# tirtho109/parallel_AMG

Measured on AMD Instinct MI355X. Metric: V-cycle iters/sec + fine-SpMV HBM GB/s, 3D Poisson 128M dofs at 1/2/4/8 GPU, higher is better.
Workload: dtype f64; 1 GPU; poisson3d 512^3 fp64, SA-AMG V(1,1) weighted-Jacobi, 1 part(s); n=134217728, nnz_fine=937951232, levels=6, max_coarse=1000, parallelism=row-slab partition p1

## Files before the change

### parallel_amg_amd/csrc/kernels.hip

```cpp

#include "pamg_device.h"
#include "div_rn.h"

namespace pamg {
namespace {

__device__ __forceinline__ int wave_incl_scan(int v) {
    const int lane = threadIdx.x & 63, rl = lane & 15;
    int t;
    t = __builtin_amdgcn_mov_dpp(v, 0x111, 0xf, 0xf, false);
    if (rl >= 1) v += t;
    t = __builtin_amdgcn_mov_dpp(v, 0x112, 0xf, 0xf, false);
    if (rl >= 2) v += t;
    t = __builtin_amdgcn_mov_dpp(v, 0x114, 0xf, 0xf, false);
    if (rl >= 4) v += t;
    t = __builtin_amdgcn_mov_dpp(v, 0x118, 0xf, 0xf, false);
    if (rl >= 8) v += t;
    t = __builtin_amdgcn_mov_dpp(v, 0x142, 0xf, 0xf, false);
    if (lane & 16) v += t;
    t = __builtin_amdgcn_mov_dpp(v, 0x143, 0xf, 0xf, false);
    if (lane >= 32) v += t;
    return v;
}

// ... 1964 lines not shown
#pragma unroll
            for (int q = 0; q < NS; ++q) {
                const int L = (int)(pw[q] & 7u);
#pragma unroll
                for (int k = 0; k < LM; ++k) {
                    const uint32_t c = (pw[q] >> (3 + 3 * k)) & 7u;
                    const int c01 = c & 1u ? an[q][0] : r[q].a0;
                    const int c23 = c & 1u ? an[q][2] : an[q][1];
                    const int c45 = c & 1u ? r[q].am : an[q][3];
                    const int c03 = c & 2u ? c23 : c01;
                    const int c47 = c & 2u ? r[q].ap : c45;
                    col[q][k] = c & 4u ? c47 : c03;
                    xv[q][k] = x[k < L ? col[q][k] : col[q][0]];
                }
            }
        };
        const int lm = 3 + (__any(lmax > 3) ? 1 : 0) + (__any(lmax > 4) ? 1 : 0) + (__any(lmax > 5) ? 1 : 0) +
                       (__any(lmax > 6) ? 1 : 0);
        switch (lm) {
            case 3: loads(std::integral_constant<int, 3>{}); break;
            case 4: loads(std::integral_constant<int, 4>{}); break;
            case 5: loads(std::integral_constant<int, 5>{}); break;
            case 6: loads(std::integral_constant<int, 6>{}); break;
            default: loads(std::integral_constant<int, 7>{}); break;
        }
#pragma unroll
        for (int q = 0; q < NS; ++q) {
            const int in = min(zs[q] + j + 1, zl[q]) * M + ixy, z2 = min(za[q] + 2, nz - 1);
            if constexpr (CP) nrec[q] = make_uint2((uint32_t)cid[in], 0u);
            else nrec[q] = rec[in];
            np0[q] = 0.0;
            np1[q] = 0.0;
            if constexpr (OP == OP_RESID || OP == OP_JACOBI) np0[q] = b[in];
            if constexpr (OP == OP_PROLONG) np0[q] = y[in];
            if constexpr (OP == OP_JACOBI) np1[q] = x[in];
            ap2[q] = anc[z2 * M + ixy];
            rg2[q] = 0;
            if (rxy >= 0) rg2[q] = anc[z2 * M + rxy];
        }
#pragma unroll
        for (int q = 0; q < NS; ++q) {
            const int i = min(zs[q] + j, zl[q]) * M + ixy, L = (int)(pw[q] & 7u);
            uint64_t rr;
            if constexpr (CP) rr = r[q].rec.x < (uint32_t)npat ? lw[r[q].rec.x] : 0ull;
            else rr = (((uint64_t)r[q].rec.y << 32) | r[q].rec.x) >> 10;
            double s = 0.0, dg = 0.0;
#pragma unroll
            for (int k = 0; k < kPncMaxLen; ++k) {
                const bool ok = k < L;
                const double v = lv[(uint32_t)(rr >> (7 * k)) & 127u];
                const double p = v * xv[q][k];
                const double t = s + p;
                s = ok ? t : s;
                if constexpr (OP == OP_JACOBI) dg = ok && col[q][k] == i ? v : dg;
            }
            double out;
            if constexpr (OP == OP_SPMV) {
                out = s;
            } else if constexpr (OP == OP_RESID) {
                out = r[q].p0 - s;
            } else if constexpr (OP == OP_JACOBI) {
                const double uu = r[q].p0 - s;
                const double v = omega * uu;
                const double w = v / dg;
                out = r[q].p1 + w;
            } else {
                out = r[q].p0 + s;
            }
            const bool in = CP ? r[q].rec.x != (uint32_t)kPncCombSkip : (r[q].rec.x & 1023u) != (uint32_t)kPncSkip;
            if (zs[q] + j < ze[q] && in) y[i] = out;
            r[q].rec = nrec[q];
            r[q].p0 = np0[q];
            r[q].p1 = np1[q];
            r[q].am = r[q].a0;
            r[q].a0 = r[q].ap;
            r[q].ap = ap2[q];
            r[q].rg = rg2[q];
            za[q] = min(za[q] + 1, nz - 1);
        }
        __syncthreads();
    }
}

template <int OP>
__global__ __launch_bounds__(kBlock) void k_rows_long(
    const int* __restrict__ rows, const int* __restrict__ rowptr, const int* __restrict__ col,
    const double* __restrict__ val, const double* __restrict__ x, const double* __restrict__ b,
    double* __restrict__ y, double omega, double c1 = 0.0, const double* __restrict__ xold = nullptr) {
    __shared__ double lprod[kBlock + 8];
    __shared__ double ldiag;
    const int tid = threadIdx.x;
    const int r = rows[blockIdx.x];
    const int z0 = rowptr[r], z1 = rowptr[r + 1];
    double s = 0.0;
    for (int base = z0; base < z1; base += kBlock) {
        const int k = base + tid;
        double p = 0.0;
        if (k < z1) {
            const int c = col[k];
            const double v = val[k];
            p = v * x[c];
            if constexpr (kDiagOp<OP>) {
                if (c == r) ldiag = v;
            }
        }
        lprod[tid] = p;
        __syncthreads();
        if (tid == 0) s = row_sum_lds(lprod, 0, min(kBlock, z1 - base), s);
        __syncthreads();
    }
    if constexpr (OP == OP_CHEB) {
        if (tid == 0) epilogue<OP>(r, s, x, b, y, omega, ldiag, c1, xold);
    } else {
        if (tid == 0) epilogue<OP>(r, s, x, b, y, omega, OP == OP_JACOBI ? ldiag : 0.0);
    }
}

__global__ __launch_bounds__(kBlock) void k_cheb_update(int64_t n, const uint8_t* __restrict__ mask, int mask_bytes,
                                                        const uint8_t* __restrict__ ids,
                                                        const uint32_t* __restrict__ mtab, uint32_t in_flag,
                                                        const double* __restrict__ diag, const double* __restrict__ x,
                                                        const double* __restrict__ xold, double* __restrict__ y,
                                                        double c1, double c2) {
    for (int64_t i = blockIdx.x * (int64_t)kBlock + threadIdx.x; i < n; i += (int64_t)gridDim.x * kBlock) {
        const uint32_t m = ids ? mtab[ids[i]]
                               : (mask_bytes == 1 ? (uint32_t)mask[i] : (uint32_t)reinterpret_cast<const uint16_t*>(mask)[i]);
        if (!(m & in_flag)) continue;
        y[i] = cheb_step(y[i], x[i], xold ? xold[i] : 0.0, diag[i], c1, c2);
    }
}

__global__ void k_jacobi_zero(int64_t n, const double* __restrict__ b,
                              const double* __restrict__ diag, double omega,
                              double* __restrict__ y) {
    for (int64_t i = blockIdx.x * (int64_t)blockDim.x + threadIdx.x; i < n;
         i += (int64_t)gridDim.x * blockDim.x) {
        const double u = b[i] - 0.0;
        const double v = omega * u;
        const double w = v / diag[i];
        y[i] = 0.0 + w;
    }
}

constexpr int kGemvChunk = 1024;
__global__ __launch_bounds__(kBlock) void k_dense_gemv(int64_t n_rows, int64_t n,
                                                       int64_t row0,
                                                       const double* __restrict__ ainv,
                                                       const double* __restrict__ b,
                                                       double* __restrict__ y) {
    __shared__ __attribute__((aligned(16))) double lp_all[kBlock / 64][kGemvChunk + 8];
    const int w = threadIdx.x >> 6, lane = threadIdx.x & 63;
    const int64_t i = (int64_t)blockIdx.x * (kBlock / 64) + w;
    if (i >= n_rows) return;
    const double* a = ainv + (row0 + i) * n;
    double* lp = lp_all[w];
    double s = 0.0;
    for (int64_t c = 0; c < n; c += kGemvChunk) {
        const int m = (int)((n - c) < kGemvChunk ? (n - c) : kGemvChunk);
#pragma unroll
        for (int q = 0; q < kGemvChunk / 64; ++q) {
            const int j = lane + 64 * q;
            if (j < m) {
                const double p = a[c + j] * b[c + j];
                lp[j] = p;
            }
        }
// ... 338 lines not shown
template <int OP>
bool launch_sym_zm(const pamg_mat& A, const double* x, const double* b, double* y, double omega, hipStream_t s,
                   Cheb ch = Cheb{}) {
    const SymDia& sd = A.sym;
    if (!(sd.nu == 3 && sd.vd_n && sd.tb_ok && !sd.tb_part && options().sym_zm && sd.plane0 == 0 &&
          (int64_t)sd.nbands * sd.band >= A.nrows && A.nrows == (int64_t)sd.tb.nx * sd.tb.ny * sd.tb.nz &&
          A.nrows % 2 == 0))
        return false;
    TbGeom g = sd.tb;
    const int tiles = g.tiles_x * g.tiles_y;
    int zc = options().zm_chunks > 0 ? options().zm_chunks : std::min((1024 + tiles - 1) / tiles, g.nz / 16);
    zc = std::max(1, std::min(zc, g.nz));
    g.zlen = (g.nz + zc - 1) / zc;
    g.zchunks = (g.nz + g.zlen - 1) / g.zlen;
    const int gr = (tiles * g.zchunks + 7) / 8 * 8;
    k_sym_zm<OP><<<gr, kZmThreads, 0, s>>>((int)A.nrows, sd.d_tid, sd.d_vtab, sd.d_mtab, sd.vd_n, g, x, b, y, omega,
                                           ch.c1, ch.xold);
    return true;
}

template <int OP, int NU>
void launch_sym_nu(const pamg_mat& A, const double* x, const double* b, double* y, double omega, hipStream_t s) {
    const SymDia& sd = A.sym;
    const int grid = sd.nbands * 8 * sd.eighth;
    if constexpr (NU == 3) {
        if (launch_sym_zm<OP>(A, x, b, y, omega, s)) return;
    }
    if (sd.vd_n) {
        const int ch = NU <= 3 ? options().symd_chunks : 1;
        const int g = 8 * ((sd.nbands * sd.eighth + ch - 1) / ch);
        if constexpr (NU <= 3) {
            if (ch == 2) {
                k_rows_symd<OP, NU, 2><<<g, kBlock, 0, s>>>((int)A.nrows, (int)A.nrows, sd.d_tid, sd.d_vtab,
                                                            sd.d_mtab, sd.vd_n, sd, x, b, y, omega);
                return;
            }
            if (ch == 4) {
                k_rows_symd<OP, NU, 4><<<g, kBlock, 0, s>>>((int)A.nrows, (int)A.nrows, sd.d_tid, sd.d_vtab,
                                                            sd.d_mtab, sd.vd_n, sd, x, b, y, omega);
                return;
            }
        }
        k_rows_symd<OP, NU><<<grid, kBlock, 0, s>>>((int)A.nrows, (int)A.nrows, sd.d_tid, sd.d_vtab, sd.d_mtab,
                                                  sd.vd_n, sd, x, b, y, omega);
        return;
    }
    if (sd.rpl == 2) {
        k_rows_sym2<OP, NU><<<grid, kBlock, 0, s>>>((int)A.nrows, (int)A.nrows, sd.d_mask, sd.d_diag, sd.d_upper,
                                                  sd.ld, sd, x, b, y, omega);
        return;
    }
    k_rows_sym<OP, NU><<<grid, kBlock, 0, s>>>((int)A.nrows, (int)A.nrows, sd.d_mask, sd.d_diag, sd.d_upper, sd.ld,
                                             sd, x, b, y, omega);
}

template <int OP>
void launch_sym(const pamg_mat& A, const double* x, const double* b, double* y, double omega, hipStream_t s,
                Cheb ch = Cheb{}) {
    if constexpr (OP == OP_PROLONG) {
        return;
    } else if constexpr (OP == OP_CHEB) {
        if (launch_sym_zm<OP_CHEB>(A, x, b, y, omega, s, ch)) return;
        launch_sym<OP_RESID>(A, x, b, y, 0.0, s);
        launch_cheb_update(A, x, ch.xold, y, ch.c1, omega, s);
    } else {
        switch (A.sym.nu) {
            case 1: launch_sym_nu<OP, 1>(A, x, b, y, omega, s); break;
            case 2: launch_sym_nu<OP, 2>(A, x, b, y, omega, s); break;
            case 3: launch_sym_nu<OP, 3>(A, x, b, y, omega, s); break;
            case 4: launch_sym_nu<OP, 4>(A, x, b, y, omega, s); break;
            case 5: launch_sym_nu<OP, 5>(A, x, b, y, omega, s); break;
            case 6: launch_sym_nu<OP, 6>(A, x, b, y, omega, s); break;
            default: launch_sym_nu<OP, 7>(A, x, b, y, omega, s); break;
        }
    }
}

constexpr int kPncZlen = 32, kPncStreams = 2;

template <int OP>
void launch_pnc(const pamg_mat& A, const double* x, const double* b, double* y, double omega, hipStream_t s) {
    const PncSet& P = A.pnc;
    const int zlen = std::min(kPncZlen, P.nz);
    const int nxb = P.nx * P.ny / 256, units = nxb * ((P.nz + zlen - 1) / zlen);
    auto go = [&](auto kern) {
        kern<<<(units + 7) / 8 * 8, 256, 0, s>>>((int)A.nrows, P.nx, P.nx * P.ny, P.nz, zlen, P.d_anc, P.d_rec, P.d_cid,
                                                P.d_pvals, P.d_ptab, P.npat, P.d_vtab, P.nval, x, b, y, omega);
    };
    if (options().pnc == 1 && pnc_tiled(P.nx, P.ny)) {
        if (P.d_cid) go(k_rows_pnct<OP, kPncStreams, true, kPncTx, kPncTy>);
        else go(k_rows_pnct<OP, kPncStreams, false, kPncTx, kPncTy>);
    } else {
        if (P.d_cid) go(k_rows_pnc<OP, kPncStreams, true>);
        else go(k_rows_pnc<OP, kPncStreams, false>);
    }
}

template <int OP>
void launch_rpat(const pamg_mat& A, const double* x, const double* b, double* y, double omega, hipStream_t s) {
    const RpatSet& R = A.rpat;
    const int grid = (int)((R.ngroups + 7) / 8 * 8);
    auto go = [&](auto kern) {
        kern<<<grid, kEllGroup, 0, s>>>((int)A.nrows, R.d_gorder, R.d_anc, R.d_pid, R.d_pmeta, R.npat, R.d_pent, R.nent,
                                        R.d_vtab, R.nval, (int)R.ngroups, x, b, y, omega);
    };
    go(k_rows_rpat<OP, 8>);
}

template <int OP, int FUSE>
void launch_bsr(const pamg_mat& A, const double* x, const double* b, double* y, double omega, hipStream_t s, Cheb ch);

template <int OP>
void launch_rows_op(const pamg_mat& A, const TileSet& ts, const double* x, const double* b,
                    double* y, double omega, hipStream_t s, Cheb ch = Cheb{}) {
    if (ts.bsr) launch_bsr<OP, 0>(A, x, b, y, omega, s, ch);
    if (ts.sym) launch_sym<OP>(A, x, b, y, omega, s, ch);
    if (ts.ell) {
        const EllSet& E = A.ell;
        const int grid = (int)((E.ngroups + 7) / 8 * 8);
        auto go = [&](auto kern) {
            kern<<<grid, kEllGroup, 0, s>>>((int)A.nrows, E.d_gorder, E.d_anc, E.d_smeta, E.d_ci, E.d_vi, E.d_len,
                                            E.d_gmeta, E.d_otab, E.d_vtab, (int)E.ngroups, x, b, y, omega, ch.c1,
                                            ch.xold);
        };
        if (E.win) {
            const int win = std::max(E.max_window, 128);
            const int gather_all = (reinterpret_cast<uintptr_t>(x) & 15) != 0 ? 1 : 0;
            const int npairs = gather_all ? 0 : E.npairs, nrest = (int)E.ngroups - 2 * npairs;
            auto gow = [&](auto kern, int span, int g0, int n, int wn) {
                const size_t bytes = sizeof(double) * (size_t)(wn + 256 * span) + sizeof(uint16_t) * 4 * 256 * span;
                kern<<<(n + 7) / 8 * 8, span * kEllGroup, bytes, s>>>(
                    (int)A.nrows, E.d_gslices, E.d_smeta, E.d_ci, E.d_cid, E.d_len, E.d_dpos, E.d_gmeta, E.d_otab,
                    E.d_vtab, E.d_wmeta, E.d_chunks, E.d_lof, wn, gather_all, E.d_pairs, g0, n, x, b, y, omega, ch.c1,
                    ch.xold);
            };
            if (npairs > 0) {
                const int wu = std::max(E.max_union, 128);
                if (E.cls) gow(k_rows_ellw<OP, true, 2>, 2, 0, npairs, wu);
                else gow(k_rows_ellw<OP, false, 2>, 2, 0, npairs, wu);
            }
            if (nrest > 0) {
                if (E.cls) gow(k_rows_ellw<OP, true>, 1, 2 * npairs, nrest, win);
                else gow(k_rows_ellw<OP, false>, 1, 2 * npairs, nrest, win);
            }
        } else if (E.d_anc) {
            if (E.paired) go(k_rows_ell<OP, true, true>);
            else go(k_rows_ell<OP, true, false>);
        } else {
            if (E.paired) go(k_rows_ell<OP, false, true>);
            else go(k_rows_ell<OP, false, false>);
        }
    }
    if constexpr (OP != OP_CHEB) {
        if (ts.pnc) launch_pnc<OP>(A, x, b, y, omega, s);
        if (ts.rpat) launch_rpat<OP>(A, x, b, y, omega, s);
    }
    if (ts.n_short > 0) {
        if (ts.tile_nnz == 1024) launch_tile<OP, 1024>(A, ts, x, b, y, omega, s, ch);
        else if (ts.tile_nnz == 4096) launch_tile<OP, 4096>(A, ts, x, b, y, omega, s, ch);
        else launch_tile<OP, 2048>(A, ts, x, b, y, omega, s, ch);
    }
    if (ts.n_long > 0)
        k_rows_long<OP><<<ts.n_long, kBlock, 0, s>>>(ts.d_long, A.d_rowptr, A.d_col, A.d_val, x,
                                                     b, y, omega, ch.c1, ch.xold);
}


__global__ __launch_bounds__(kBlock) void k_pcg_alpha(int np, const double* __restrict__ partials, PcgScalars* S) {
    if (S->done) return;
    __shared__ double lds[kBlock / 64];
    double v = 0.0;
    for (int i = threadIdx.x; i < np; i += kBlock) v += partials[i];
    const double s = block_sum(v, lds);
    if (threadIdx.x == 0) {
        S->pq = s;
        S->alpha = S->rz / s;
    }
// ... 339 lines not shown
```

### parallel_amg_amd/csrc/matrix.hip

```cpp
#include <algorithm>
#include <array>
#include <atomic>
#include <chrono>
#include <cstdint>
#include <cstdio>
#include <cstdlib>
#include <cstring>
#include <functional>
#include <iterator>
#include <memory>
#include <mutex>
#include <new>
#include <thread>
#include <utility>
#include <vector>

#include "pamg_device.h"
#include "pamg_host.h"
#include "ell_span.h"

namespace {

int host_threads() {
    static const int n = [] {
// ... 91 lines not shown
    int dev = 0, cus = 0;
    if (hipGetDevice(&dev) != hipSuccess ||
        hipDeviceGetAttribute(&cus, hipDeviceAttributeMultiprocessorCount, dev) != hipSuccess || cus <= 0)
        return 256;
    return cus;
}

std::vector<int> column_reuse_gaps(const PtrVec& rp, const IdxVec& ci, int64_t nrows,
                                   int64_t ncols) {
    std::vector<int> gap(ncols, 0);
    const int nch = (int)std::min<int64_t>(host_threads(), std::max<int64_t>(1, nrows / 65536));
    std::vector<int64_t> r0(nch + 1);
    for (int t = 0; t <= nch; ++t) r0[t] = nrows * t / nch;
    auto each_chunk = [nch](const std::function<void(int)>& f) {
        std::vector<std::thread> th;
        for (int t = 0; t < nch; ++t) th.emplace_back([&f, t] { f(t); });
        for (auto& x : th) x.join();
    };
    std::vector<int> lo(nch, INT32_MAX), hi(nch, -1);
    each_chunk([&](int t) {
        int a = INT32_MAX, b = -1;
        for (int64_t k = rp[r0[t]]; k < rp[r0[t + 1]]; ++k)
            if (ci[k] < ncols) {
                a = std::min(a, ci[k]);
                b = std::max(b, ci[k]);
            }
        lo[t] = a;
        hi[t] = b;
    });
    int64_t span = 0;
    for (int t = 0; t < nch; ++t) span += hi[t] >= lo[t] ? (int64_t)hi[t] - lo[t] + 1 : 0;
    if (nch == 1 || span > 2 * ncols + 65536) {
        std::vector<int> last(ncols, -1);
        for (int64_t i = 0; i < nrows; ++i)
            for (int64_t k = rp[i]; k < rp[i + 1]; ++k) {
                const int c = ci[k];
                if (c < ncols) {
                    if (last[c] >= 0) gap[c] = std::max(gap[c], (int)i - last[c]);
                    last[c] = (int)i;
                }
            }
        return gap;
    }
    std::vector<std::vector<int>> first(nch), last(nch), cgap(nch);
    each_chunk([&](int t) {
        if (hi[t] < lo[t]) return;
        const int64_t w = (int64_t)hi[t] - lo[t] + 1;
        first[t].assign(w, -1);
        last[t].assign(w, -1);
        cgap[t].assign(w, 0);
        int* f = first[t].data();
        int* l = last[t].data();
        int* g = cgap[t].data();
        for (int64_t i = r0[t]; i < r0[t + 1]; ++i)
            for (int64_t k = rp[i]; k < rp[i + 1]; ++k) {
                const int c = ci[k];
                if (c >= ncols) continue;
                const int j = c - lo[t];
                if (l[j] >= 0) g[j] = std::max(g[j], (int)i - l[j]);
                else f[j] = (int)i;
                l[j] = (int)i;
            }
    });
    par_for(ncols, [&](int64_t a, int64_t b) {
        for (int64_t c = a; c < b; ++c) {
            int g = 0, prev = -1;
            for (int t = 0; t < nch; ++t) {
                if (c < lo[t] || c > hi[t]) continue;
                const int64_t j = c - lo[t];
                if (first[t][j] < 0) continue;
                if (prev >= 0) g = std::max(g, first[t][j] - prev);
                g = std::max(g, cgap[t][j]);
                prev = last[t][j];
            }
            gap[c] = g;
        }
    });
    return gap;
}

std::vector<std::array<int64_t, 4>> grids_of(pamg_ctx* ctx) {
    std::lock_guard<std::mutex> lk(ctx->grids_mu);
    return ctx->grids;
}

int blocked_group_order(pamg_ctx* ctx, const std::vector<int>& anc, int64_t ng, int64_t own_cols, int** d_order) {
    using pamg::kEllGroup;
    const int yb = pamg::options().ell_yblock;
    for (const auto& gr : grids_of(ctx))
        if (yb > 0 && gr[0] == own_cols) {
            const int64_t gnx = gr[1], gny = gr[2], gM = gr[1] * gr[2];
            std::vector<int64_t> key(ng);
            par_for(ng, [&](int64_t a, int64_t b) {
                for (int64_t g = a; g < b; ++g) {
                    const int64_t c = anc[g * kEllGroup];
                    const int64_t y = (c / gnx) % gny, z = c / gM;
                    key[g] = ((y / yb) << 40) | (z << 20) | y;
                }
            });
            const int64_t per = (ng + 7) / 8;
            std::vector<int> order(ng);
            for (int64_t g = 0; g < ng; ++g) order[g] = (int)g;
            for (int64_t e = 0; e < 8; ++e) {
                const int64_t lo = std::min(ng, e * per), hi = std::min(ng, (e + 1) * per);
                std::stable_sort(order.begin() + lo, order.begin() + hi, [&](int p, int q) { return key[p] < key[q]; });
            }
            CHECK(dalloc(d_order, ng));
            CHECK(h2d(ctx, *d_order, order.data(), sizeof(int) * ng));
            break;
        }
    return PAMG_OK;
}

struct Upload {
    pamg_mat* A;
    const PtrVec& rp;
    const IdxVec& ci;
    const double* val;
    int64_t n_own_cols;
    bool has_all_diag;
    std::vector<int>& inner;
    const std::vector<int>& bnd;
    const std::function<int64_t()>& band;
    UploadTrace& tr;
    int bs = 1;
    bool rect = false;
};


int build_sym_dia(pamg_mat* A, const PtrVec& rp, const IdxVec& ci, const double* val,
                  const std::vector<int>& inner, const std::function<int64_t()>& get_band) {
    using pamg::kSymMaxU;
    const int64_t n = A->nrows;
    constexpr int kMaxOff = 2 * kSymMaxU + 1;
    std::mutex mu;
    std::vector<int> offs;
    std::atomic<bool> too_many{false};
    par_for((int64_t)inner.size(), [&](int64_t a, int64_t b) {
        std::vector<int> loc;
        for (int64_t q = a; q < b && !too_many; ++q) {
            const int i = inner[q];
            for (int64_t k = rp[i]; k < rp[i + 1]; ++k) {
                const int o = ci[k] - i;
                if (std::find(loc.begin(), loc.end(), o) == loc.end()) {
                    loc.push_back(o);
                    if ((int)loc.size() > kMaxOff) {
                        too_many = true;
                        return;
                    }
                }
            }
        }
        std::lock_guard<std::mutex> g(mu);
        for (int o : loc)
            if (std::find(offs.begin(), offs.end(), o) == offs.end()) offs.push_back(o);
    });
    if (too_many || (int)offs.size() > kMaxOff) return PAMG_OK;
    std::sort(offs.begin(), offs.end());
    const int no = (int)offs.size();
    if (no % 2 == 0 || offs[no / 2] != 0) return PAMG_OK;
    for (int k = 0; k < no; ++k)
        if (offs[k] != -offs[no - 1 - k]) return PAMG_OK;
    const int nu = no / 2;
    if (nu < 1) return PAMG_OK;
    pamg::SymDia sd;
    sd.nu = nu;
// ... 102 lines not shown
            std::vector<std::thread> th;
            for (int c = 0; c < nch; ++c)
                th.emplace_back([&, c] {
                    std::vector<Key>& f = firsts[c];
                    int last = -1;
                    for (int64_t i = n * c / nch, e = n * (c + 1) / nch; i < e && !over; ++i) {
                        const Key k = key_of(i);
                        if (last >= 0 && f[last] == k) continue;
                        last = -1;
                        for (int q = 0; q < (int)f.size() && last < 0; ++q)
                            if (f[q] == k) last = q;
                        if (last >= 0) continue;
                        if ((int)f.size() == pamg::kSymVdMax) {
                            over = true;
                            break;
                        }
                        f.push_back(k);
                        last = (int)f.size() - 1;
                    }
                });
            for (auto& x : th) x.join();
        }
        std::vector<Key> tab;
        for (int c = 0; c < nch && !over; ++c)
            for (const Key& k : firsts[c]) {
                if (std::find(tab.begin(), tab.end(), k) != tab.end()) continue;
                if ((int)tab.size() == pamg::kSymVdMax) {
                    over = true;
                    break;
                }
                tab.push_back(k);
            }
        if (!over && !tab.empty()) {
            tid.assign(n + kVecPad, 0);
            par_for(n, [&](int64_t a, int64_t b) {
                int last = 0;
                for (int64_t i = a; i < b; ++i) {
                    const Key k = key_of(i);
                    if (tab[last] != k) last = (int)(std::find(tab.begin(), tab.end(), k) - tab.begin());
                    tid[i] = (uint8_t)last;
                }
            });
            const int nv = (int)tab.size();
            vtab.assign((size_t)nv * (nu + 1) + kVecPad, 0.0);
            mtab.assign(nv + kVecPad, 0u);
            for (int e = 0; e < nv; ++e) {
                mtab[e] = (uint32_t)tab[e][0];
                for (int c = 0; c <= nu; ++c) std::memcpy(&vtab[(size_t)e * (nu + 1) + c], &tab[e][1 + c], 8);
            }
            sd.vd_n = nv;
            std::vector<int64_t> cnt(nv, 0);
            {
                std::mutex mu;
                par_for(n, [&](int64_t a, int64_t b) {
                    std::vector<int64_t> c(nv, 0);
                    for (int64_t i = a; i < b; ++i) ++c[tid[i]];
                    std::lock_guard<std::mutex> lk(mu);
                    for (int e = 0; e < nv; ++e) cnt[e] += c[e];
                });
            }
            sd.vd_main = (int)(std::max_element(cnt.begin(), cnt.end()) - cnt.begin());
        }
    }
    if (sd.vd_n) {
        CHECK(dalloc(&sd.d_tid, (int64_t)tid.size()));
        CHECK(h2d(A->ctx, sd.d_tid, tid.data(), tid.size()));
        CHECK(dalloc(&sd.d_vtab, (int64_t)vtab.size()));
        CHECK(h2d(A->ctx, sd.d_vtab, vtab.data(), sizeof(double) * vtab.size()));
        CHECK(dalloc(&sd.d_mtab, (int64_t)mtab.size()));
        CHECK(h2d(A->ctx, sd.d_mtab, mtab.data(), sizeof(uint32_t) * mtab.size()));
    } else {
        CHECK(dalloc(&sd.d_mask, (n + kVecPad) * mb));
        CHECK(dalloc(&sd.d_diag, n + kVecPad));
        CHECK(dalloc(&sd.d_upper, (int64_t)nu * sd.ld));
        if (mb == 1) {
            std::vector<uint8_t> m8(mask.begin(), mask.end());
            CHECK(h2d(A->ctx, sd.d_mask, m8.data(), m8.size()));
        } else {
            CHECK(h2d(A->ctx, sd.d_mask, mask.data(), sizeof(uint16_t) * mask.size()));
        }
        CHECK(h2d(A->ctx, sd.d_diag, dg.data(), sizeof(double) * dg.size()));
        CHECK(h2d(A->ctx, sd.d_upper, up.data(), sizeof(double) * up.size()));
    }
    part = part && sd.band == Mp;
    if (nu == 3 && mb == 1 && (whole || part) && sd.off[0] == 1 && sd.off[2] % sd.off[1] == 0 && n % sd.off[2] == 0) {
        const int nx = sd.off[1], ny = sd.off[2] / sd.off[1];
        const int nz = (int)(n / sd.off[2]);
        bool ok = nx % pamg::kTbX == 0 && ny % pamg::kTbY == 0;
        std::atomic<bool> cross{false};
        if (ok)
            par_for(n, [&](int64_t a0, int64_t b0) {
                for (int64_t i = a0; i < b0 && !cross; ++i) {
                    const int x = (int)(i % nx), y = (int)((i / nx) % ny);
                    const uint32_t m = mask[i];
                    if (((m & 4u) && x == 0) || ((m & 16u) && x == nx - 1) || ((m & 2u) && y == 0) ||
                        ((m & 32u) && y == ny - 1))
                        cross = true;
                }
            });
        if (ok && !cross) {
            pamg::TbGeom& g = sd.tb;
            g.nx = nx;
            g.ny = ny;
            g.nz = nz;
            g.tiles_x = nx / pamg::kTbX;
            g.tiles_y = ny / pamg::kTbY;
            const int tiles = g.tiles_x * g.tiles_y;
            const int want = std::max(1, (device_cus() + tiles - 1) / tiles);
            g.zchunks = std::max(1, std::min(want, nz / 4 > 0 ? nz / 4 : 1));
            g.zlen = (nz + g.zchunks - 1) / g.zchunks;
            g.zchunks = (nz + g.zlen - 1) / g.zlen;
            g.zlo = 0;
            g.zhi = nz;
            sd.tb_ok = whole;
            sd.tb_part = part;
            if (whole || part) {
                const std::array<int64_t, 4> gk{n, nx, ny, nz};
                std::lock_guard<std::mutex> lk(A->ctx->grids_mu);
                auto& gs = A->ctx->grids;
                if (std::find(gs.begin(), gs.end(), gk) == gs.end()) gs.push_back(gk);
            }
            sd.part_lo = part ? plo : 0;
            sd.part_hi = part ? phi : nz;
        }
    }
    A->sym = sd;
    A->interior.sym = true;
    A->interior.rows_short = (int64_t)inner.size();
    return PAMG_OK;
}

int sym_try(Upload& u) {
    pamg_mat* A = u.A;
    if (pamg::options().sym_dia && u.n_own_cols == A->nrows && u.has_all_diag && !u.inner.empty())
        CHECK(build_sym_dia(A, u.rp, u.ci, u.val, u.inner, u.band));
    if (A->interior.sym) u.inner.clear();
    u.tr.mark("sym dia");
    return PAMG_OK;
}

void sym_free(pamg::SymDia& S) {
    dfree(S.d_mask);
    dfree(S.d_diag);
    dfree(S.d_upper);
    dfree(S.d_tid);
    dfree(S.d_vtab);
    dfree(S.d_mtab);
    S = pamg::SymDia{};
}

int64_t sym_bytes(const pamg_mat* A) {
    if (!A->interior.sym) return 0;
    const int64_t nrows = A->nrows;
    return A->sym.vd_n ? nrows + (int64_t)A->sym.vd_n * (8 * (A->sym.nu + 1) + 4)
                       : nrows * (A->sym.mask_bytes + 8 + 8 * (int64_t)A->sym.nu);
}

void sym_report(const pamg_mat* A, const pamg::TileSet& t, int out[10]) {
    if (!t.sym) return;
    out[4] = A->sym.nu;
    out[8] = A->sym.nbands * 8 * A->sym.eighth;
    out[9] |= 8 | (A->sym.rpl == 2 ? 16 : 0) | (A->sym.tb_ok || A->sym.tb_part ? 32 : 0) | (A->sym.vd_n ? 128 : 0);
}


int build_rpat(pamg_mat* A, const PtrVec& rp, const IdxVec& ci, const double* val, const std::vector<int>& inner) {
    using pamg::kRpatEnt;
    using pamg::kRpatMax;
    using pamg::kRpatMaxLen;
    using pamg::kRpatSkip;
    const int64_t n = A->nrows;
    if (n <= 0) return PAMG_OK;
    std::vector<char> in_set;
    if ((int64_t)inner.size() != n) {
        in_set.assign(n, 0);
        for (int i : inner) in_set[i] = 1;
    }
    auto member = [&](int64_t i) { return in_set.empty() || in_set[i]; };
    auto row_hash = [&](int64_t i) {
        uint64_t h = 0x9E3779B97F4A7C15ull ^ (uint64_t)(rp[i + 1] - rp[i]);
        const int64_t c0 = ci[rp[i]];
        for (int64_t k = rp[i]; k < rp[i + 1]; ++k) {
            uint64_t u;
            std::memcpy(&u, &val[k], 8);
            h = (h ^ (uint64_t)(ci[k] - c0)) * 0x100000001B3ull;
            h = (h ^ u) * 0x9E3779B97F4A7C15ull;
            h ^= h >> 29;
        }
        return h;
    };
    auto same = [&](int64_t i, int64_t j) {
        const int64_t L = rp[i + 1] - rp[i];
        if (L != rp[j + 1] - rp[j]) return false;
        const int64_t ci0 = ci[rp[i]], cj0 = ci[rp[j]];
        for (int64_t k = 0; k < L; ++k) {
            if (ci[rp[i] + k] - ci0 != ci[rp[j] + k] - cj0) return false;
            if (std::memcmp(&val[rp[i] + k], &val[rp[j] + k], 8) != 0) return false;
        }
        return true;
    };
    const int nch = std::max(1, std::min<int>(host_threads() * 4, (int)(n / 65536)));
    std::vector<std::vector<std::pair<uint64_t, int64_t>>> firsts(nch);
    std::atomic<bool> ok{true};
    {
        std::vector<std::thread> th;
        const int nt = std::min(nch, host_threads());
// ... 2360 lines not shown
```

### parallel_amg_amd/csrc/runtime.hip

```cpp
#include <dlfcn.h>

#include <algorithm>
#include <atomic>
#include <chrono>
#include <cmath>
#include <condition_variable>
#include <cstddef>
#include <cstdint>
#include <cstdio>
#include <cstring>
#include <limits>
#include <memory>
#include <mutex>
#include <optional>
#include <string>
#include <thread>
#include <utility>
#include <vector>

#include "cycle_plan.h"
#include "multi_cols.h"
#include "pamg_device.h"
#include "pamg_host.h"

// ... 2174 lines not shown
        const bool replay = H->use_graph && !H->prof && H->g_pcg[0] && H->g_pcg[1];
        auto half = [&](int h) -> int {
            if (replay) HIPC(hipGraphLaunch(H->g_pcg[h], s));
            else CHECK(pcg_half_enqueue(H, xd, h));
            return PAMG_OK;
        };
        const int ring = lookahead + 1;
        volatile const int* slot = H->pcg_slot;
        for (int j = 1; j <= maxit; ++j) {
            CHECK(half(0));
            ++enq;
            HIPC(hipEventRecord(H->pcg_ev[j % ring], s));
            if (lookahead == 0) {
                HIPC(hipEventSynchronize(H->pcg_ev[j % ring]));
                if (slot[1]) break;
                CHECK(half(1));
                continue;
            }
            CHECK(half(1));
            if (j > lookahead) {
                HIPC(hipEventSynchronize(H->pcg_ev[(j - lookahead) % ring]));
                if (slot[1]) break;
            }
        }
    }
    d.finish(x);
    HIPC(hipGetLastError());
    HIPC(hipStreamSynchronize(s));
    if (enq > 0) {
        HIPC(hipMemcpy(&k, &H->pcg_S->k, sizeof(int), hipMemcpyDeviceToHost));
        if (k < 0 || k > enq) return fail(PAMG_E_STATE, "pcg_resident: iteration counter %d of %d enqueued", k, enq);
    }
    if (res_hist) {
        res_hist[0] = nr0;
        if (k > 0) {
            HIPC(hipMemcpy(res_hist + 1, H->pcg_hist + 1, sizeof(double) * k, hipMemcpyDeviceToHost));
            for (int i = 1; i <= k; ++i) res_hist[i] = std::sqrt(res_hist[i]);
        }
    }
    if (iters) *iters = k;
    if (stats) {
        stats[0] = enq;
        stats[1] = enq - k;
    }
    return PAMG_OK;
}

}

namespace {
struct OptionRow {
    const char* key;
    int pamg::Options::*member;
    int64_t lo, hi;
    bool pow2;
};
using O = pamg::Options;
const OptionRow kOptionTable[] = {
    {"tile_nnz", &O::tile_nnz, 1024, 4096, true},
    {"tile_order", &O::tile_order, 0, 1, false},
    {"poison_ghosts", &O::poison_ghosts, 0, 1, false},
    {"col24", &O::col24, 0, 1, false},
    {"long_tiles", &O::long_tiles, 0, 1, false},
    {"row_len8", &O::row_len8, 0, 1, false},
    {"value_dict", &O::value_dict, 0, 2, false},
    {"col_dict", &O::col_dict, 0, 1, false},
    {"tile_major", &O::tile_major, 0, 2, false},
    {"col_dict_anchor", &O::col_dict_anchor, 0, 1, false},
    {"col_dict_tile", &O::col_dict_tile, 0, 1, false},
    {"x_stage", &O::x_stage, 0, 1, false},
    {"band_pct", &O::band_pct, 1, 10000, false},
    {"band_pct_restrict", &O::band_pct_restrict, 1, 10000, false},
    {"long_tiles_min", &O::long_tiles_min, 1, 255, false},
    {"tm_tile_dicts", &O::tm_tile_dicts, 0, 1, false},
    {"sym_dia", &O::sym_dia, 0, 1, false},
    {"sym_rows", &O::sym_rows, 1, 2, false},
    {"jr_fuse", &O::jr_fuse, 0, 1, false},
    {"sym_vd", &O::sym_vd, 0, 1, false},
    {"symd_chunks", &O::symd_chunks, 1, 4, true},
    {"sym_zm", &O::sym_zm, 0, 1, false},
    {"tb_xfast", &O::tb_xfast, 0, 1, false},
    {"ell", &O::ell, 0, 1, false},
    {"ell_restrict", &O::ell_restrict, 0, 1, false},
    {"pnc", &O::pnc, 0, 2, false},
    {"rpat", &O::rpat, 0, 1, false},
    {"pnc_compact", &O::pnc_compact, 0, 1, false},
    {"ell_pair", &O::ell_pair, 0, 1, false},
    {"ell_xwin", &O::ell_xwin, 0, 4, false},
    {"ell_xwin_max", &O::ell_xwin_max, 2, pamg::kEllWinCap, false},
    {"ell_yblock", &O::ell_yblock, 0, 65536, false},
    {"ell_min_rows", &O::ell_min_rows, 0, INT32_MAX, false},
    {"zm_chunks", &O::zm_chunks, 0, 4096, false},
    {"chain_store_x", &O::chain_store_x, 0, 1, false},
};

const OptionRow* find_option(const char* key) {
    for (const OptionRow& r : kOptionTable)
        if (std::strcmp(r.key, key) == 0) return &r;
    return nullptr;
}
}

extern "C" {

int pamg_set_option(const char* key, int64_t value) {
    if (!key) return fail(PAMG_E_ARG, "set_option: NULL key");
    const OptionRow* r = find_option(key);
    if (!r || value < r->lo || value > r->hi || (r->pow2 && (value & (value - 1)) != 0))
        return fail(PAMG_E_ARG, "set_option: unknown key or bad value: %s=%lld", key, (long long)value);
    pamg::options().*(r->member) = (int)value;
    return PAMG_OK;
}

int pamg_get_option(const char* key, int64_t* value) {
    if (!key || !value) return fail(PAMG_E_ARG, "get_option: bad args");
    const OptionRow* r = find_option(key);
    if (!r) return fail(PAMG_E_ARG, "get_option: unknown key %s", key);
    *value = pamg::options().*(r->member);
    return PAMG_OK;
}

int pamg_hier_bench_chain(pamg_hier* H, pamg_vec* x, const pamg_vec* b, int reps, double* avg_ms) {
    if (!H || !x || !b || reps < 1 || !avg_ms) return fail(PAMG_E_ARG, "hier_bench_chain: bad args");
    if (!pipe_ok(H, 2, false)) return fail(PAMG_E_STATE, "hier_bench_chain: the hierarchy does not run the cross-cycle pipeline");
    pamg_ctx* ctx = H->ctx;
    CHECK(check_vec_for(H->A[0], x, "hier_bench_chain"));
    CHECK(set_device(ctx));
    CHECK(ensure_u0(H));
    int k = -1;
    return time_reps(ctx->s_comp, reps, avg_ms, [&]() {
        const bool back = k > 0 && (k & 1);
        ++k;
        return launch_chain3(H, x->d, b->d, back ? H->u0 : H->t[0], back ? H->t[0] : H->u0);
    });
}

int pamg_bench_rowop(pamg_ctx* ctx, const pamg_mat* A, int op, pamg_vec* x, const pamg_vec* b,
                     pamg_vec* y, double omega, int reps, double* avg_ms) {
    if (!ctx || !A || !x || !y || reps < 1 || !avg_ms || op < 0 || op > 6)
        return fail(PAMG_E_ARG, "bench_rowop: bad args");
    if ((op == pamg::OP_RESID || op == pamg::OP_JACOBI || op >= 4) && !b) return fail(PAMG_E_ARG, "bench_rowop: b needed");
    if ((op == pamg::OP_JACOBI || op >= 4) && !A->d_diag)
        return fail(PAMG_E_SETUP, "bench_rowop: jacobi needs a square matrix");
    if (op == pamg::OP_CHEB) {
        if (A->interior.pnc || A->interior.rpat) return fail(PAMG_E_ARG, "bench_rowop: op 6 needs a square operator");
        if (x == y || b == y) return fail(PAMG_E_ARG, "bench_rowop: y must differ from x and b");
        CHECK(check_vec_for(A, x, "bench_rowop"));
        if (b->n_own != A->nrows || y->n_own != A->nrows) return fail(PAMG_E_ARG, "bench_rowop: size mismatch");
        CHECK(set_device(ctx));
        double* xo = nullptr;
        CHECK(dalloc(&xo, A->nrows + kVecPad));
        int rc = dzero(ctx, xo, sizeof(double) * (size_t)(A->nrows + kVecPad));
        hipStream_t s = ctx->s_comp;
        if (rc == PAMG_OK)
            rc = time_reps(s, reps, avg_ms, [&]() {
                pamg::launch_rows(*A, A->interior, op, x->d, b->d, xo, y->d, omega, s, omega);
                pamg::launch_rows(*A, A->boundary, op, x->d, b->d, xo, y->d, omega, s, omega);
                return PAMG_OK;
            });
        dfree(xo);
        return rc;
    }
    if (op >= 4 && !(A->interior.sym && (A->sym.tb_ok || A->sym.tb_part)))
        return fail(PAMG_E_STATE, "bench_rowop: op %d needs the temporally blocked layout (pamg_mat_layout bit 5)", op);
    if (op == pamg::OP_PROLONG && (A->interior.sym || A->boundary.sym))
        return fail(PAMG_E_STATE, "bench_rowop: the symmetric layouts have no prolongate-add kernel");
    if (x == y) return fail(PAMG_E_ARG, "bench_rowop: x and y must differ");
// ... 524 lines not shown
```

Before: 234.7 V-cycles/s.

## Add register-and-LDS z-stencil PNC kernel with LDS pattern/value tables

Adds k_rows_pncv, a tiled pattern-compressed SpMV/residual/prolong kernel. It stages each z-plane's x values for a tile plus its halo ring in double-buffered LDS, keeps z-1/z+1 neighbours in registers, and decodes pattern offsets into LDS byte offsets, so it no longer gathers x through the anchor and column indices for every nonzero. Pattern and value tables move to dynamic LDS. This kernel becomes the default for non-Jacobi ops when pnc==1 and the grid is tiled, with a new mode 3 keeping the old tiled kernel. Grid registration also now covers slab partitions and 2D 5-point grids, which can enable tiled paths elsewhere. The cost is extra LDS use and a barrier per z-step.

```diff
diff --git a/parallel_amg_amd/csrc/kernels.hip b/parallel_amg_amd/csrc/kernels.hip
--- a/parallel_amg_amd/csrc/kernels.hip
+++ b/parallel_amg_amd/csrc/kernels.hip
@@ -2070,6 +2070,167 @@
     }
 }
 
+struct PncvRow {
+    uint2 rec;
+    double p0;
+    double em, e0, ep;
+    int a2;
+    double gp;
+    int ga2;
+};
+
+template <int OP, int NS, bool CP, int TX, int TY>
+__global__ __launch_bounds__(TX * TY) void k_rows_pncv(int nrows, int nx, int M, int nz, int zlen,
+                                                       const int* __restrict__ anc, const uint2* __restrict__ rec,
+                                                       const uint16_t* __restrict__ cid, const uint64_t* __restrict__ pvals,
+                                                       const uint32_t* __restrict__ ptab, int npat,
+                                                       const double* __restrict__ vtab, int nval,
+                                                       const double* __restrict__ x, const double* __restrict__ b,
+                                                       double* __restrict__ y, double omega) {
+    constexpr int NT = TX * TY, LW = TX + 2, LP = LW * (TY + 2);
+    static_assert(OP != OP_JACOBI, "the diagonal test needs the columns: k_rows_pnct");
+    static_assert(NT % 64 == 0 && NT <= 1024 && 2 * TX + 2 * TY <= NT, "one row per lane; one ring point per edge thread");
+    __shared__ double le[NS][2][LP];
+    extern __shared__ double pncv_tab[];
+    double* lv = pncv_tab;
+    uint64_t* lw = reinterpret_cast<uint64_t*>(pncv_tab + max(nval, 1));
+    uint2* lo = reinterpret_cast<uint2*>(lw + (CP ? npat : 0));
+    static_assert(LW > 2 && LW < 128, "a pattern's LDS offsets are signed bytes; +-2 name the z neighbours");
+    const int nxb = M / NT;
+    const int units = nxb * ((nz + zlen - 1) / zlen);
+    const int per = (units + 7) >> 3;
+    const int u = (int)(blockIdx.x & 7) * per + (int)(blockIdx.x >> 3);
+    if (u >= units) return;
+    const int tid = (int)threadIdx.x;
+    for (int t = tid; t < npat; t += NT) {
+        const uint32_t w = ptab[t];
+        uint32_t o[2] = {0u, (w & 7u) << 24};
+#pragma unroll
+        for (int k = 0; k < kPncMaxLen; ++k) {
+            const uint32_t c = (w >> (3 + 3 * k)) & 7u;
+            const int e = c == 1u ? -1 : c == 2u ? 1 : c == 3u ? -LW : c == 4u ? LW : c == 5u ? 2 : c == 6u ? -2 : 0;
+            o[k >> 2] |= ((uint32_t)e & 255u) << (8 * (k & 3));
+        }
+        lo[t] = make_uint2(o[0], o[1]);
+    }
+    if constexpr (CP)
+        for (int t = tid; t < npat; t += NT) lw[t] = pvals[t];
+    for (int t = tid; t < nval; t += NT) lv[t] = vtab[t];
+    const int zc0 = (u / nxb) * zlen, zc1 = min(nz, zc0 + zlen);
+    const int part = (zc1 - zc0 + NS - 1) / NS;
+    const int tpx = nx / TX, ny = M / nx, tb = u % nxb;
+    const int x0 = (tb % tpx) * TX, y0 = (tb / tpx) * TY;
+    const int ixy = (y0 + tid / TX) * nx + x0 + tid % TX;
+    const int lpos = (tid / TX + 1) * LW + tid % TX + 1;
+    int rxy = -1, rpos = 0;
+    if (tid < TX) {
+        rxy = (y0 > 0 ? y0 - 1 : y0) * nx + x0 + tid;
+        rpos = tid + 1;
+    } else if (tid < 2 * TX) {
+        rxy = (y0 + TY < ny ? y0 + TY : y0 + TY - 1) * nx + x0 + tid - TX;
+        rpos = (TY + 1) * LW + tid - TX + 1;
+    } else if (tid >= NT - TY) {
+        rxy = (y0 + tid - (NT - TY)) * nx + (x0 + TX < nx ? x0 + TX : x0 + TX - 1);
+        rpos = (tid - (NT - TY) + 1) * LW + TX + 1;
+    } else if (tid >= NT - 2 * TY) {
+        rxy = (y0 + tid - (NT - 2 * TY)) * nx + (x0 > 0 ? x0 - 1 : x0);
+        rpos = (tid - (NT - 2 * TY) + 1) * LW;
+    }
+    int zs[NS], ze[NS], zl[NS], za[NS];
+    PncvRow r[NS];
+#pragma unroll
+    for (int q = 0; q < NS; ++q) {
+        zs[q] = zc0 + q * part;
+        ze[q] = min(zc1, zs[q] + part);
+        zl[q] = ze[q] > zs[q] ? ze[q] - 1 : zc1 - 1;
+        const int z = za[q] = min(zs[q], zl[q]), zp = min(z + 1, nz - 1), z2 = min(z + 2, nz - 1), i = z * M + ixy;
+        if constexpr (CP) r[q].rec = make_uint2((uint32_t)cid[i], 0u);
+        else r[q].rec = rec[i];
+        r[q].p0 = 0.0;
+        if constexpr (OP == OP_RESID) r[q].p0 = b[i];
+        if constexpr (OP == OP_PROLONG) r[q].p0 = y[i];
+        r[q].e0 = x[anc[i]];
+        r[q].em = x[anc[z > 0 ? i - M : i]];
+        r[q].ep = x[anc[zp * M + ixy]];
+        r[q].a2 = anc[z2 * M + ixy];
+        r[q].gp = 0.0;
+        r[q].ga2 = 0;
+        le[q][0][lpos] = r[q].e0;
+        if (rxy >= 0) {
+            le[q][0][rpos] = x[anc[z * M + rxy]];
+            r[q].gp = x[anc[zp * M + rxy]];
+            r[q].ga2 = anc[z2 * M + rxy];
+        }
+    }
+    __syncthreads();
+    for (int j = 0; j < part; ++j) {
+        uint2 ow[NS];
+#pragma unroll
+        for (int q = 0; q < NS; ++q) {
+            const uint32_t pid = CP ? r[q].rec.x : r[q].rec.x & 1023u;
+            ow[q] = pid < (uint32_t)npat ? lo[pid] : make_uint2(0u, 0u);
+            le[q][(j & 1) ^ 1][lpos] = r[q].ep;
+            if (rxy >= 0) le[q][(j & 1) ^ 1][rpos] = r[q].gp;
+        }
+        uint2 nrec[NS];
+        double np0[NS], e2[NS], g2[NS];
+        int a3[NS], ga3[NS];
+#pragma unroll
+        for (int q = 0; q < NS; ++q) {
+            const int in = min(zs[q] + j + 1, zl[q]) * M + ixy, z3 = min(za[q] + 3, nz - 1);
+            if constexpr (CP) nrec[q] = make_uint2((uint32_t)cid[in], 0u);
+            else nrec[q] = rec[in];
+            np0[q] = 0.0;
+            if constexpr (OP == OP_RESID) np0[q] = b[in];
+            if constexpr (OP == OP_PROLONG) np0[q] = y[in];
+            e2[q] = x[r[q].a2];
+            a3[q] = anc[z3 * M + ixy];
+            g2[q] = 0.0;
+            ga3[q] = 0;
+            if (rxy >= 0) {
+                g2[q] = x[r[q].ga2];
+                ga3[q] = anc[z3 * M + rxy];
+            }
+        }
+#pragma unroll
+        for (int q = 0; q < NS; ++q) {
+            const int i = min(zs[q] + j, zl[q]) * M + ixy, L = (int)(ow[q].y >> 24);
+            uint64_t rr;
+            if constexpr (CP) rr = r[q].rec.x < (uint32_t)npat ? lw[r[q].rec.x] : 0ull;
+            else rr = (((uint64_t)r[q].rec.y << 32) | r[q].rec.x) >> 10;
+            const double* pl = &le[q][j & 1][lpos];
+            double s = 0.0;
+#pragma unroll
+            for (int k = 0; k < kPncMaxLen; ++k) {
+                if (k < L) {
+                    const int o = (int)((k < 4 ? ow[q].x : ow[q].y) << (24 - 8 * (k & 3))) >> 24;
+                    const double ei = pl[o];
+                    const double xv = o == 2 ? r[q].em : o == -2 ? r[q].ep : ei;
+                    const double v = lv[(uint32_t)(rr >> (7 * k)) & 127u];
+                    const double p = v * xv;
+                    s = s + p;
+                }
+            }
+            double out;
+            if constexpr (OP == OP_SPMV) out = s;
+            else if constexpr (OP == OP_RESID) out = r[q].p0 - s;
+            else out = r[q].p0 + s;
+            const bool in = CP ? r[q].rec.x != (uint32_t)kPncCombSkip : (r[q].rec.x & 1023u) != (uint32_t)kPncSkip;
+            if (zs[q] + j < ze[q] && in) y[i] = out;
+            r[q].rec = nrec[q];
+            r[q].p0 = np0[q];
+            r[q].em = r[q].e0;
+            r[q].e0 = r[q].ep;
+            r[q].ep = e2[q];
+            r[q].a2 = a3[q];
+            r[q].gp = g2[q];
+            r[q].ga2 = ga3[q];
+            za[q] = min(za[q] + 1, nz - 1);
+        }
+        __syncthreads();
+    }
+}
+
 template <int OP>
 __global__ __launch_bounds__(kBlock) void k_rows_long(
     const int* __restrict__ rows, const int* __restrict__ rowptr, const int* __restrict__ col,
@@ -2574,17 +2735,26 @@
 void launch_pnc(const pamg_mat& A, const double* x, const double* b, double* y, double omega, hipStream_t s) {
     const PncSet& P = A.pnc;
     const int zlen = std::min(kPncZlen, P.nz);
-    const int nxb = P.nx * P.ny / 256, units = nxb * ((P.nz + zlen - 1) / zlen);
-    auto go = [&](auto kern) {
-        kern<<<(units + 7) / 8 * 8, 256, 0, s>>>((int)A.nrows, P.nx, P.nx * P.ny, P.nz, zlen, P.d_anc, P.d_rec, P.d_cid,
-                                                P.d_pvals, P.d_ptab, P.npat, P.d_vtab, P.nval, x, b, y, omega);
+    const int chunks = (P.nz + zlen - 1) / zlen;
+    auto go = [&](auto kern, int nt, size_t lds) {
+        const int units = P.nx * P.ny / nt * chunks;
+        kern<<<(units + 7) / 8 * 8, nt, lds, s>>>((int)A.nrows, P.nx, P.nx * P.ny, P.nz, zlen, P.d_anc, P.d_rec, P.d_cid,
+                                                 P.d_pvals, P.d_ptab, P.npat, P.d_vtab, P.nval, x, b, y, omega);
     };
-    if (options().pnc == 1 && pnc_tiled(P.nx, P.ny)) {
-        if (P.d_cid) go(k_rows_pnct<OP, kPncStreams, true, kPncTx, kPncTy>);
-        else go(k_rows_pnct<OP, kPncStreams, false, kPncTx, kPncTy>);
+    const size_t tab = sizeof(double) * std::max(P.nval, 1) + (P.d_cid ? 16 : 8) * (size_t)P.npat;
+    const int mode = options().pnc;
+    const bool tiled = pnc_tiled(P.nx, P.ny);
+    if (OP != OP_JACOBI && mode == 1 && tiled) {
+        if constexpr (OP != OP_JACOBI) {
+            if (P.d_cid) go(k_rows_pncv<OP, kPncStreams, true, kPncTx, kPncTy>, kPncTx * kPncTy, tab);
+            else go(k_rows_pncv<OP, kPncStreams, false, kPncTx, kPncTy>, kPncTx * kPncTy, tab);
+        }
+    } else if ((mode == 1 || mode == 3) && tiled) {
+        if (P.d_cid) go(k_rows_pnct<OP, kPncStreams, true, kPncTx, kPncTy>, 256, 0);
+        else go(k_rows_pnct<OP, kPncStreams, false, kPncTx, kPncTy>, 256, 0);
     } else {
-        if (P.d_cid) go(k_rows_pnc<OP, kPncStreams, true>);
-        else go(k_rows_pnc<OP, kPncStreams, false>);
+        if (P.d_cid) go(k_rows_pnc<OP, kPncStreams, true>, 256, 0);
+        else go(k_rows_pnc<OP, kPncStreams, false>, 256, 0);
     }
 }
 
diff --git a/parallel_amg_amd/csrc/matrix.hip b/parallel_amg_amd/csrc/matrix.hip
--- a/parallel_amg_amd/csrc/matrix.hip
+++ b/parallel_amg_amd/csrc/matrix.hip
@@ -197,6 +197,13 @@
 std::vector<std::array<int64_t, 4>> grids_of(pamg_ctx* ctx) {
     std::lock_guard<std::mutex> lk(ctx->grids_mu);
     return ctx->grids;
+}
+
+void register_grid(pamg_ctx* ctx, int64_t n, int64_t nx, int64_t ny, int64_t nz) {
+    const std::array<int64_t, 4> gk{n, nx, ny, nz};
+    std::lock_guard<std::mutex> lk(ctx->grids_mu);
+    auto& gs = ctx->grids;
+    if (std::find(gs.begin(), gs.end(), gk) == gs.end()) gs.push_back(gk);
 }
 
 int blocked_group_order(pamg_ctx* ctx, const std::vector<int>& anc, int64_t ng, int64_t own_cols, int** d_order) {
@@ -465,13 +472,14 @@
         CHECK(h2d(A->ctx, sd.d_diag, dg.data(), sizeof(double) * dg.size()));
         CHECK(h2d(A->ctx, sd.d_upper, up.data(), sizeof(double) * up.size()));
     }
+    const bool slab = part;
     part = part && sd.band == Mp;
-    if (nu == 3 && mb == 1 && (whole || part) && sd.off[0] == 1 && sd.off[2] % sd.off[1] == 0 && n % sd.off[2] == 0) {
+    if (nu == 3 && mb == 1 && (whole || slab) && sd.off[0] == 1 && sd.off[2] % sd.off[1] == 0 && n % sd.off[2] == 0) {
         const int nx = sd.off[1], ny = sd.off[2] / sd.off[1];
         const int nz = (int)(n / sd.off[2]);
-        bool ok = nx % pamg::kTbX == 0 && ny % pamg::kTbY == 0;
+        const bool ok = nx % pamg::kTbX == 0 && ny % pamg::kTbY == 0, reg = ok || pamg::pnc_tiled(nx, ny);
         std::atomic<bool> cross{false};
-        if (ok)
+        if (reg)
             par_for(n, [&](int64_t a0, int64_t b0) {
                 for (int64_t i = a0; i < b0 && !cross; ++i) {
                     const int x = (int)(i % nx), y = (int)((i / nx) % ny);
@@ -481,7 +489,7 @@
                         cross = true;
                 }
             });
-        if (ok && !cross) {
+        if (ok && !cross && (whole || part)) {
             pamg::TbGeom& g = sd.tb;
             g.nx = nx;
             g.ny = ny;
@@ -497,14 +505,24 @@
             g.zhi = nz;
             sd.tb_ok = whole;
             sd.tb_part = part;
-            if (whole || part) {
-                const std::array<int64_t, 4> gk{n, nx, ny, nz};
-                std::lock_guard<std::mutex> lk(A->ctx->grids_mu);
-                auto& gs = A->ctx->grids;
-                if (std::find(gs.begin(), gs.end(), gk) == gs.end()) gs.push_back(gk);
-            }
             sd.part_lo = part ? plo : 0;
             sd.part_hi = part ? phi : nz;
+        }
+        if (reg && !cross) register_grid(A->ctx, n, nx, ny, nz);
+    } else if (nu == 2 && mb == 1 && whole && sd.off[0] == 1 && n % sd.off[1] == 0) {
+        const int nx = sd.off[1], ny = (int)(n / sd.off[1]);
+        std::atomic<bool> cross{false};
+        if (pamg::pnc_tiled(nx, ny)) {
+            par_for(n, [&](int64_t a0, int64_t b0) {
+                for (int64_t i = a0; i < b0 && !cross; ++i) {
+                    const int x = (int)(i % nx), y = (int)(i / nx);
+                    const uint32_t m = mask[i];
+                    if (((m & 2u) && x == 0) || ((m & 8u) && x == nx - 1) || ((m & 1u) && y == 0) ||
+                        ((m & 16u) && y == ny - 1))
+                        cross = true;
+                }
+            });
+            if (!cross) register_grid(A->ctx, n, nx, ny, 1);
         }
     }
     A->sym = sd;
diff --git a/parallel_amg_amd/csrc/runtime.hip b/parallel_amg_amd/csrc/runtime.hip
--- a/parallel_amg_amd/csrc/runtime.hip
+++ b/parallel_amg_amd/csrc/runtime.hip
@@ -2280,7 +2280,7 @@
     {"tb_xfast", &O::tb_xfast, 0, 1, false},
     {"ell", &O::ell, 0, 1, false},
     {"ell_restrict", &O::ell_restrict, 0, 1, false},
-    {"pnc", &O::pnc, 0, 2, false},
+    {"pnc", &O::pnc, 0, 3, false},
     {"rpat", &O::rpat, 0, 1, false},
     {"pnc_compact", &O::pnc_compact, 0, 1, false},
     {"ell_pair", &O::ell_pair, 0, 1, false},
```

New measurement: 242.8 V-cycles/s, median of 6. 3.5% higher.
